# s0phia-/tetris

Hardware: AMD Instinct MI355X
Metric: env-steps/sec (higher is better)
Workload: dtype u32; 1 GPU; 1048576 envs/GPU x 1 GPU, 10x20 board, pieces=default, uniform random valid actions, in-kernel auto-reset, device bag seed 0; envs_per_gpu=1048576, observation_output=True, env_steps_per_launch=1, steps_per_graph_replay=1, streams_per_gpu=1, board=10x20, pieces=default, backend=single, device=cuda

## Files before the change

### tetris_amd/csrc/tetris_core.hpp

```cpp
#pragma once
#include <stdint.h>

#if defined(__HIPCC__)
#include <hip/hip_runtime.h>
#define TET_HD __host__ __device__ __forceinline__
#else
#define TET_HD inline
#endif

#ifndef TET_ABLATE
#define TET_ABLATE 0
#endif
#ifndef TET_BAG_SMALL_PATH
#define TET_BAG_SMALL_PATH 1
#endif
#ifndef TET_RESCUE_SKIP
#define TET_RESCUE_SKIP 1
#endif

#ifndef TET_FENCE_EVERY
#define TET_FENCE_EVERY 2
#endif
#ifndef TET_FENCE_MASK
#define TET_FENCE_MASK 1
#endif
#if defined(__HIP_DEVICE_COMPILE__)
#define TET_SCHED_FENCE() __builtin_amdgcn_sched_barrier(0)
#define TET_PIN(x) asm volatile("" : "+v"(x))
#else
#define TET_SCHED_FENCE() ((void)0)
#define TET_PIN(x) ((void)0)
#endif

#if defined(__HIP_DEVICE_COMPILE__)
#define TET_WAVE_ANY(x) (__ballot((x)) != 0ull)
#else
#define TET_WAVE_ANY(x) (x)
#endif

#if defined(__HIP_DEVICE_COMPILE__)
#define TET_SCRATCH_OR(ptr, v) ((void)__hip_atomic_fetch_or((ptr), (v), __ATOMIC_RELAXED, __HIP_MEMORY_SCOPE_WORKGROUP))
#else
#define TET_SCRATCH_OR(ptr, v) (*(ptr) |= (v))
#endif

#if defined(__HIP_DEVICE_COMPILE__)
#define TET_FMUL(a, b) __fmul_rn((a), (b))
#define TET_FADD(a, b) __fadd_rn((a), (b))
#else
#define TET_FMUL(a, b) ((float)((volatile float)(a) * (b)))
#define TET_FADD(a, b) ((float)((volatile float)(a) + (b)))
#endif

namespace tet {

constexpr int kMaxPieces = 12;
constexpr int kMaxCols = 12;
constexpr int kNumCatalogue = 9;

struct Orient {
  int w, H, b[4], n[4];
  bool exists;
};

TET_HD Orient unpack_orient(uint32_t d) {
  Orient o;
  o.w = d & 7;
  o.H = (d >> 3) & 7;
#pragma unroll
  for (int j = 0; j < 4; ++j) {
    o.b[j] = (d >> (6 + 5 * j)) & 3;
    o.n[j] = (d >> (8 + 5 * j)) & 7;
  }
  o.exists = (d >> 31) != 0;
  return o;
}

#ifndef TET_NO_PACK
#define TET_NO_PACK 0
#endif
TET_HD constexpr bool board_packed(int word_bytes, int num_rows) { return !TET_NO_PACK && num_rows + 4 <= 6 * word_bytes; }
TET_HD constexpr int n_planes(int C, bool packed) { return packed ? (C / 4) * 3 + ((C % 4) * 3 + 3) / 4 : C; }
constexpr int kTileEnvs = 64;
TET_HD constexpr int64_t plane_index(int64_t i, int p, int NP) { return ((i >> 6) * NP + p) * kTileEnvs + (i & 63); }
TET_HD constexpr int64_t board_words(int64_t B, int NP) { return ((B + kTileEnvs - 1) / kTileEnvs) * NP * kTileEnvs; }

template <typename W, int C, bool PACK>
TET_HD void unpack_board(const W (&w)[n_planes(C, PACK)], W (&col)[C]) {
  if (!PACK) {
#pragma unroll
    for (int c = 0; c < C; ++c) col[c] = w[c < n_planes(C, PACK) ? c : 0];
    return;
  }
  constexpr int Wb = 8 * (int)sizeof(W), F = Wb * 3 / 4, P = n_planes(C, PACK);
  const W M = (W)(((W)1 << F) - 1);
#pragma unroll
  for (int g = 0; 4 * g < C; ++g) {
    const int b = 3 * g, c0 = 4 * g;
    const W w0 = w[b], w1 = w[b + 1 < P ? b + 1 : b], w2 = w[b + 2 < P ? b + 2 : b];
    col[c0] = (W)(w0 & M);
    if (c0 + 1 < C) col[c0 + 1] = (W)(((w0 >> F) | (w1 << (Wb - F))) & M);
    if (c0 + 2 < C) col[c0 + 2] = (W)(((w1 >> (2 * F - Wb)) | (w2 << (2 * Wb - 2 * F))) & M);
    if (c0 + 3 < C) col[c0 + 3] = (W)(w2 >> (3 * F - 2 * Wb));
  }
}

template <typename W, int C, bool PACK>
TET_HD void pack_board(const W (&col)[C], W (&w)[n_planes(C, PACK)]) {
  if (!PACK) {
#pragma unroll
    for (int c = 0; c < n_planes(C, PACK); ++c) w[c] = col[c < C ? c : 0];
    return;
  }
  constexpr int Wb = 8 * (int)sizeof(W), F = Wb * 3 / 4, P = n_planes(C, PACK);
#pragma unroll
  for (int g = 0; 4 * g < C; ++g) {
    const int b = 3 * g, c0 = 4 * g;
    const W x0 = col[c0], x1 = c0 + 1 < C ? col[c0 + 1 < C ? c0 + 1 : c0] : (W)0;
    const W x2 = c0 + 2 < C ? col[c0 + 2 < C ? c0 + 2 : c0] : (W)0, x3 = c0 + 3 < C ? col[c0 + 3 < C ? c0 + 3 : c0] : (W)0;
    w[b] = (W)(x0 | (x1 << F));
    if (b + 1 < P) w[b + 1 < P ? b + 1 : b] = (W)((x1 >> (Wb - F)) | (x2 << (2 * F - Wb)));
    if (b + 2 < P) w[b + 2 < P ? b + 2 : b] = (W)((x2 >> (2 * Wb - 2 * F)) | (x3 << (3 * F - 2 * Wb)));
  }
}

template <typename W, int C, bool PACK>
TET_HD void load_board(const W* planes, int64_t , int64_t i, W (&col)[C]) {
  constexpr int NP = n_planes(C, PACK);
  W w[NP];
  const W* rec = planes + plane_index(i, 0, NP);
#pragma unroll
  for (int p = 0; p < NP; ++p) w[p] = rec[p * kTileEnvs];
  unpack_board<W, C, PACK>(w, col);
}
template <typename W, int C, bool PACK>
TET_HD void store_board(W* planes, int64_t , int64_t i, const W (&col)[C]) {
  constexpr int NP = n_planes(C, PACK);
  W w[NP];
  pack_board<W, C, PACK>(col, w);
  W* rec = planes + plane_index(i, 0, NP);
#pragma unroll
  for (int p = 0; p < NP; ++p) rec[p * kTileEnvs] = w[p];
}

template <typename W>
TET_HD W load_column_rt(const W* planes, int64_t , int64_t i, int c, int C, bool packed) {
  const int NP = n_planes(C, packed);
  if (!packed) return planes[plane_index(i, c, NP)];
  constexpr int Wb = 8 * (int)sizeof(W), F = Wb * 3 / 4;
  const W M = (W)(((W)1 << F) - 1);
  const int b = 3 * (c >> 2), k = c & 3;
  const W lo = planes[plane_index(i, b + (k == 0 ? 0 : k - 1), NP)];
  if (k == 0) return (W)(lo & M);
  if (k == 3) return (W)(lo >> (3 * F - 2 * Wb));
  const W hi = planes[plane_index(i, b + k, NP)];
  return k == 1 ? (W)(((lo >> F) | (hi << (Wb - F))) & M) : (W)(((lo >> (2 * F - Wb)) | (hi << (2 * Wb - 2 * F))) & M);
}
template <typename W>
TET_HD void store_columns_rt(W* planes, int64_t , int64_t i, const W* col, int C, bool packed) {
  if (!packed) {
    for (int c = 0; c < C; ++c) planes[plane_index(i, c, C)] = col[c];
    return;
  }
  constexpr int Wb = 8 * (int)sizeof(W), F = Wb * 3 / 4;
  const int P = n_planes(C, true);
  for (int p = 0; p < P; ++p) {
    const int c0 = 4 * (p / 3), q = p % 3;
    const W a = c0 + q < C ? col[c0 + q] : (W)0, b = c0 + q + 1 < C ? col[c0 + q + 1] : (W)0;
    const W v = q == 0 ? (W)(a | (b << F))
                       : (q == 1 ? (W)((a >> (Wb - F)) | (b << (2 * F - Wb))) : (W)((a >> (2 * Wb - 2 * F)) | (b << (3 * F - 2 * Wb))));
    planes[plane_index(i, p, P)] = v;
  }
}

constexpr uint64_t kMaskBits = (1ull << 48) - 1;
constexpr int kFieldStride = 12;
TET_HD constexpr int mask_bit(int k, int c) { return kFieldStride * k + c; }
TET_HD uint64_t meta_pack(uint64_t mask, int piece, uint32_t bag) {
  return (mask & kMaskBits) | ((uint64_t)(piece & 15) << 48) | ((uint64_t)(bag & 0xFFF) << 52);
}
TET_HD uint64_t meta_mask(uint64_t m) { return m & kMaskBits; }
TET_HD int meta_piece(uint64_t m) { return (int)((m >> 48) & 15); }
TET_HD uint32_t meta_bag(uint64_t m) { return (uint32_t)(m >> 52); }

TET_HD int popc(uint32_t x) { return __builtin_popcount(x); }
TET_HD int popc(uint64_t x) { return __builtin_popcountll(x); }
TET_HD int bitlen(uint32_t x) { return 31 - __builtin_clz((x << 1) | 1u); }
TET_HD int bitlen(uint64_t x) { return 63 - __builtin_clzll((x << 1) | 1ull); }
template <typename W>
TET_HD W lowmask(int n) { return (W)(((W)1 << n) - 1); }

TET_HD uint32_t mix32(uint32_t x) {
  x ^= x >> 16;
  x *= 0x7feb352dU;
  x ^= x >> 15;
  x *= 0x846ca68bU;
  x ^= x >> 16;
  return x;
}
TET_HD uint32_t hash_key(uint64_t seed, uint64_t counter) {
  uint32_t k = mix32((uint32_t)seed ^ 0x9E3779B9U);
  k = mix32(k ^ (uint32_t)(seed >> 32));
  k = mix32(k ^ (uint32_t)counter);
  k = mix32(k ^ (uint32_t)(counter >> 32));
  return k;
}
TET_HD uint32_t hash_env(uint32_t key, uint32_t env) {
  uint32_t h = (key ^ env) * 0x9E3779B1U;
  h ^= h >> 16;
  h *= 0x85EBCA6BU;
  h ^= h >> 13;
  return h;
}
TET_HD int scale16(uint32_t r16, int n) { return (int)((r16 * (uint32_t)n) >> 16); }

TET_HD int select_bit32(uint32_t v, int k) {
  int pos = 0;
  int c = popc(v & 0xFFFFu);
  if (k >= c) { k -= c; pos += 16; v >>= 16; }
  c = popc(v & 0xFFu);
  if (k >= c) { k -= c; pos += 8; v >>= 8; }
  c = popc(v & 0xFu);
  if (k >= c) { k -= c; pos += 4; v >>= 4; }
  c = popc(v & 0x3u);
  if (k >= c) { k -= c; pos += 2; v >>= 2; }
  c = (int)(v & 1u);
  if (k >= c) { pos += 1; }
  return pos;
}
TET_HD int bag_draw(uint32_t& bag, int n_pieces, uint32_t r16) {
  if (bag == 0) bag = (1u << n_pieces) - 1u;
  const int k = scale16(r16, popc(bag));
  uint32_t v = bag;
  int pos = 0;
  int c = popc(v & 0xFFu);
  if (k >= c) { pos = 8; v >>= 8; }
  int kk = k >= c ? k - c : k;
  c = popc(v & 0xFu);
  if (kk >= c) { kk -= c; pos += 4; v >>= 4; }
  c = popc(v & 0x3u);
  if (kk >= c) { kk -= c; pos += 2; v >>= 2; }
  c = (int)(v & 1u);
  if (kk >= c) pos += 1;
  bag &= ~(1u << pos);
  return pos;
}

TET_HD int bag_draw_lut(uint32_t& bag, int n_pieces, uint32_t r16, const uint8_t* sel_nib) {
  if (bag == 0) bag = (1u << n_pieces) - 1u;
#if TET_BAG_SMALL_PATH
  if (n_pieces <= 4) {
    const int k4 = scale16(r16, popc(bag));
    const int pos4 = (int)sel_nib[bag * 4u + (uint32_t)k4];
    bag &= ~(1u << pos4);
    return pos4;
  }
#endif
  int k = scale16(r16, popc(bag));
  const int c0 = popc(bag & 0xFu), c1 = c0 + popc(bag & 0xF0u);
  const int grp = (k >= c0) + (k >= c1);
  k -= grp == 0 ? 0 : (grp == 1 ? c0 : c1);
  const uint32_t nib = (bag >> (4 * grp)) & 15u;
  const int pos = 4 * grp + (int)sel_nib[nib * 4u + (uint32_t)k];
  bag &= ~(1u << pos);
  return pos;
}

struct alignas(16) OrientEntry {
  uint32_t sh[4];
  uint32_t rj0[2];
  uint32_t rj1[2];
  uint32_t vert4;
  uint32_t desc;
  uint32_t pad_[2];
};
static_assert(sizeof(OrientEntry) == 48, "table staging and LDS reads assume 48-byte entries");

struct SetTable {
  OrientEntry orient[kMaxPieces][4];
  uint64_t fullmask[kMaxPieces];
};

TET_HD const OrientEntry* piece_entries(const SetTable& tab, int np) {
  uint32_t off = (uint32_t)np * (uint32_t)sizeof(tab.orient[0]);
  TET_PIN(off);
  return reinterpret_cast<const OrientEntry*>(reinterpret_cast<const char*>(&tab.orient[0][0]) + off);
}

template <int CR>
struct LutLayout {
  static constexpr int kHoleEntries = 1 << (CR + 1), kWellsEntries = 1 << CR;
  static constexpr int kHoleA = 0, kHoleU = kHoleEntries, kWellsS = 2 * kHoleEntries;
  static constexpr int kWellsLead = kWellsS + kWellsEntries, kWellsTrail = kWellsLead + kWellsEntries;
  static constexpr int kSelPair = kWellsTrail + kWellsEntries, kSelNib = kSelPair + 256 * 8;
  static constexpr int kBytes = kSelNib + 16 * 4;
};
constexpr int kFeatureLutBytes = LutLayout<12>::kBytes;
constexpr int kFeatureLut10Bytes = LutLayout<10>::kBytes;
struct AfterLut {
  static constexpr int kHoleA = LutLayout<12>::kHoleA, kHoleU = LutLayout<12>::kHoleU;
  static constexpr int kWellsPack = 2 * LutLayout<12>::kHoleEntries;
  static constexpr int kSelPair = kWellsPack + 4 * LutLayout<12>::kWellsEntries, kSelNib = kSelPair + 256 * 8;
  static constexpr int kBytes = kSelNib + 16 * 4;
};
constexpr int kAfterLutBytes = AfterLut::kBytes;

TET_HD uint32_t spread2(uint32_t x) {
  x = (x | (x << 8)) & 0x00FF00FFu;
  x = (x | (x << 4)) & 0x0F0F0F0Fu;
  x = (x | (x << 2)) & 0x33333333u;
  x = (x | (x << 1)) & 0x55555555u;
  return x;
}

template <int C>
TET_HD uint32_t mask_field(uint64_t mask, int k) { return (uint32_t)(mask >> (kFieldStride * k)) & ((1u << C) - 1u); }

template <int C>
TET_HD void slot_of_action_lut(uint64_t mask, int k, const uint8_t* sel_pair, int& kk, int& c) {
  static_assert(C <= 12, "three 4-column groups per 12-bit field");
  constexpr uint32_t kLoopBits = (1u << (2 * kFieldStride)) - 1u;
  const uint32_t w0 = (uint32_t)mask & kLoopBits, w1 = (uint32_t)(mask >> (2 * kFieldStride)) & kLoopBits;
  const int n0 = popc(w0);
  const bool second = k >= n0;
  const uint32_t w = second ? w1 : w0;
  int kr = second ? k - n0 : k;
  constexpr uint32_t kG0 = 0xFu | (0xFu << kFieldStride);
  const int c0 = popc(w & kG0), c1 = c0 + popc(w & (kG0 << 4));
  const int grp = (C > 4 ? (kr >= c0) : 0) + (C > 8 ? (kr >= c1) : 0);
  kr -= grp == 0 ? 0 : (grp == 1 ? c0 : c1);
  const uint32_t t = w >> (4 * grp);
  const uint32_t idx = (t & 15u) | (((t >> kFieldStride) & 15u) << 4);
  const uint32_t r = sel_pair[idx * 8u + (uint32_t)kr];
  c = 4 * grp + (int)(r & 3u);
  kk = (second ? 2 : 0) + (int)(r >> 2);
}
template <int C>
TET_HD void slot_of_action(uint64_t mask, int k, int& kk, int& c) {
  const uint32_t f0 = mask_field<C>(mask, 0), f1 = mask_field<C>(mask, 1);
  const uint32_t f2 = mask_field<C>(mask, 2), f3 = mask_field<C>(mask, 3);
  const int n0 = popc(f0) + popc(f1);
  const bool second = k >= n0;
  const uint32_t z = spread2(second ? f2 : f0) | (spread2(second ? f3 : f1) << 1);
  const int pos = select_bit32(z, second ? k - n0 : k);
  c = pos >> 1;
  kk = (second ? 2 : 0) + (pos & 1);
}
template <int C>
TET_HD int row_of_slot(uint64_t mask, int kk, int c) {
  const int L = kk >> 1;
  const uint32_t fa = mask_field<C>(mask, 2 * L), fb = mask_field<C>(mask, 2 * L + 1);
  const uint32_t below = (1u << c) - 1u;
  int row = popc(fa & below) + popc(fb & below) + ((kk & 1) ? (int)((fa >> c) & 1u) : 0);
  if (L) row += popc(mask_field<C>(mask, 0)) + popc(mask_field<C>(mask, 1));
  return row;
}

template <typename W, int C>
TET_HD void heights_of(const W (&col)[C], int (&h)[C]) {
#pragma unroll
  for (int c = 0; c < C; ++c) h[c] = bitlen(col[c]);
}

template <typename W, int C>
TET_HD int stamp_static(const W (&col)[C], const int (&h)[C], int c, const Orient& o, W (&nb)[C],
                        W (&pbits)[4]) {
  int a = -64;
#pragma unroll
  for (int j = 0; j < 4; ++j)
    if (c + j < C) {
      int v = (j < o.w) ? h[c + j] - o.b[j] : -64;
      a = v > a ? v : a;
    }
  if (a < 0) a = 0;
#pragma unroll
  for (int i = 0; i < C; ++i) nb[i] = col[i];
#pragma unroll
  for (int j = 0; j < 4; ++j) {
    int nj = (j < o.w) ? o.n[j] : 0;
    pbits[j] = (W)(lowmask<W>(nj) << (a + o.b[j]));
    if (c + j < C) nb[c + j] |= pbits[j];
  }
  return a;
}

template <typename W, int C>
TET_HD int clear_lines(W (&col)[C], const W (&pbits)[4], int a, int* eroded_cells) {
  W F = (W)((W)~(W)0 << a);
#pragma unroll
  for (int i = 0; i < C; ++i) F &= col[i];
  int k = popc(F);
  int er = 0;
  if (F != 0) {
#pragma unroll
    for (int j = 0; j < 4; ++j) er += popc((W)(F & pbits[j]));
    while (F != 0) {
      int p = bitlen(F) - 1;
      W low = lowmask<W>(p);
#pragma unroll
      for (int i = 0; i < C; ++i) col[i] = (W)((col[i] & low) | ((col[i] >> (p + 1)) << p));
      F = (W)(F & low);
    }
  }
  *eroded_cells = er;
  return k;
}

template <typename W, int NCH = 0, int CR = 12>
TET_HD void col_own(W x, int hi, int R, const uint8_t* lut, W& ho, int& nh, int& f1, int& f7) {
  ho = (W)(~x & lowmask<W>(hi));
  nh = popc(ho);
  const uint8_t* lut_a = lut + LutLayout<CR>::kHoleA;
  const uint8_t* lut_u = lut + LutLayout<CR>::kHoleU;
  int d7 = 0, u = 0;
  if (!(TET_ABLATE & 16)) {
#pragma unroll
    for (int k = 0; CR * k < (int)(8 * sizeof(W)) - 1; ++k) {
      if (NCH > 0 ? k < NCH : (k < 2 || CR * k < R + 4)) {
        const uint32_t up = (uint32_t)(x >> (CR * k));
        const uint32_t idx = (NCH > 0 && k == NCH - 1) ? up : (up & (uint32_t)(LutLayout<CR>::kHoleEntries - 1));
        const int uk = lut_u[idx];
        u += uk;
        d7 += lut_a[idx];
        const bool more = NCH > 0 ? k + 1 < NCH : (CR * (k + 1) < R + 4);
        if (CR * (k + 1) < (int)(8 * sizeof(W)) && more) d7 += uk * popc((W)(x >> (CR * (k + 1))));
      }
    }
  }
  f1 = 2 * u;
  f7 = d7;
}

template <typename W>
TET_HD int col_rowtrans(W x, W L, int hi, int hL, int nh_left) {
  const int dl = hL - hi;
  return popc((W)((x ^ L) & lowmask<W>(hi))) + (dl > 0 ? dl : 0) - ((hi == 0) ? nh_left : 0);
}

template <typename W, int NCH = 0, int CR = 12>
TET_HD int col_wells(W x, W L, W Rr, int hi, int R, bool left_wall, bool right_wall, const uint8_t* lut) {
  W w = (W)(~x & L & Rr);
  if (left_wall || right_wall) w = (W)(w & lowmask<W>(hi > R ? hi : R));
  const uint8_t* lut_s = lut + LutLayout<CR>::kWellsS;
  const uint8_t* lut_lead = lut + LutLayout<CR>::kWellsLead;
  const uint8_t* lut_trail = lut + LutLayout<CR>::kWellsTrail;
  int total = 0, carry = 0;
#pragma unroll
  for (int k = 0; CR * k < (int)(8 * sizeof(W)) - 1; ++k) {
    if (NCH > 0 ? k < NCH : (k < 2 || CR * k < R + 4)) {
      const uint32_t up = (uint32_t)(w >> (CR * k));
      const uint32_t idx = (NCH > 0 && k == NCH - 1) ? up : (up & (uint32_t)(LutLayout<CR>::kWellsEntries - 1));
      const bool last = NCH > 0 && k == NCH - 1;
      total += lut_s[idx];
      if (k == 0) {
        if (!last) carry = lut_trail[idx];
      } else {
        const int lead = lut_lead[idx];
        total += carry * lead;
        if (!last) {
          const int trail = lut_trail[idx];
          carry = (lead == CR) ? carry + CR : trail;
        }
      }
    }
  }
  return (TET_ABLATE & 32) ? 0 : total;
}

template <typename W, int NCH = 0>
TET_HD int col_wells_packed(W x, W L, W Rr, int hi, int R, bool left_wall, bool right_wall, const uint32_t* pack) {
  constexpr int CR = 12;
  W w = (W)(~x & L & Rr);
  if (left_wall || right_wall) w = (W)(w & lowmask<W>(hi > R ? hi : R));
  uint32_t total = 0, carry = 0;
#pragma unroll
  for (int k = 0; CR * k < (int)(8 * sizeof(W)) - 1; ++k) {
    if (NCH > 0 ? k < NCH : (k < 2 || CR * k < R + 4)) {
      const uint32_t up = (uint32_t)(w >> (CR * k));
      const bool last = NCH > 0 && k == NCH - 1;
      const uint32_t e = pack[last ? up : (up & 4095u)];
      total += e & 0xFFFFu;
      const uint32_t lead = e >> 24, trail = (e >> 16) & 255u;
      if (k == 0) {
        if (!last) carry = trail;
      } else {
        total += carry * lead;
        if (!last) carry = (lead == (uint32_t)CR) ? carry + (uint32_t)CR : trail;
      }
    }
  }
  return (int)total;
}

template <typename W, int C, int NCH = 0, int CR = 12, bool PACKW = false>
TET_HD void board_features(const W (&col)[C], const int (&h)[C], int R, const uint8_t* hole_lut,
                           int& rows_with_holes, int& col_trans, int& holes, int& wells, int& row_trans,
                           int& hole_depth) {
  const W wall = lowmask<W>(R + 4);
  W hole_rows = 0;
  int f1 = C;
  int f2 = 0, f4 = 0, f7 = 0;
  int f5 = R - popc(col[C - 1]);
  int nh_left = 0;
#pragma unroll
  for (int i = 0; i < C; ++i) {
    const W L = (i == 0) ? wall : col[i - 1];
    const W Rr = (i == C - 1) ? wall : col[i + 1];
    const int hL = (i == 0) ? R : h[i - 1];
    W ho;
    int nh, d1, d7;
    col_own<W, NCH, CR>(col[i], h[i], R, hole_lut, ho, nh, d1, d7);
    f1 += d1;
    f2 += nh;
    f7 += d7;
    hole_rows |= ho;
    f5 += col_rowtrans<W>(col[i], L, h[i], hL, nh_left);
    nh_left = nh;
    if (PACKW)
      f4 += col_wells_packed<W, NCH>(col[i], L, Rr, h[i], R, i == 0, i == C - 1,
                                     reinterpret_cast<const uint32_t*>(hole_lut + AfterLut::kWellsPack));
    else
      f4 += col_wells<W, NCH, CR>(col[i], L, Rr, h[i], R, i == 0, i == C - 1, hole_lut);
    if (TET_FENCE_EVERY > 0 && i % TET_FENCE_EVERY == TET_FENCE_EVERY - 1 && i + 1 < C) {
      TET_PIN(f1);
      TET_PIN(f2);
      TET_PIN(f4);
      TET_PIN(f5);
      TET_PIN(f7);
      TET_SCHED_FENCE();
    }
  }
  rows_with_holes = popc(hole_rows);
  col_trans = f1;
  holes = f2;
  wells = f4;
  row_trans = f5;
  hole_depth = f7;
}

template <typename W, int C, int NCH = 0, int CR = 12, bool PACKW = false>
TET_HD void bcts_features(const W (&col)[C], const int (&h)[C], int R, const uint8_t* hole_lut, int anchor_row,
                          int H, int eroded_cells, int n_cleared, float (&f)[8]) {
  int f0, f1, f2, f4, f5, f7;
  board_features<W, C, NCH, CR, PACKW>(col, h, R, hole_lut, f0, f1, f2, f4, f5, f7);
  f[0] = (float)f0;
  f[1] = (float)f1;
  f[2] = (float)f2;
  f[3] = (float)anchor_row + 0.5f * (float)(H - 1) + 1.0f;
  f[4] = (float)f4;
  f[5] = (float)f5;
  f[6] = (float)(eroded_cells * n_cleared);
  f[7] = (float)f7;
}

TET_HD constexpr int level_stride(int C) { return C <= 10 ? 10 : 12; }
template <int C> struct MissBits { typedef uint32_t type; };
template <> struct MissBits<11> { typedef uint64_t type; };
template <> struct MissBits<12> { typedef uint64_t type; };
TET_HD int ctz_any(uint32_t x) { return __builtin_ctz(x); }
TET_HD int ctz_any(uint64_t x) { return __builtin_ctzll(x); }

template <typename W, int C>
TET_HD uint64_t valid_mask(const W (&col)[C], const int (&h)[C], const OrientEntry* tab, uint64_t fullmask, int R) {
  static_assert(C <= 12, "four 12-bit level fields + one empty field fill the 64-bit level word; 12-bit mask fields");
  constexpr int LS = level_stride(C);
  typedef typename MissBits<C>::type FT;
  uint32_t P[3] = {0u, 0u, 0u};
#pragma unroll
  for (int c = 0; c < C; ++c) P[c >> 2] |= (uint32_t)h[c] << (8 * (c & 3));
  uint32_t lv[4];
#pragma unroll
  for (int l = 1; l <= 4; ++l) {
    const uint32_t K = (uint32_t)(127 - (R - l)) * 0x01010101u;
    uint32_t g = 0;
#pragma unroll
    for (int q = 0; q < (C + 3) / 4; ++q)
      g |= ((((P[q] + K) & 0x80808080u) * 0x00204081u) >> 28) << (4 * q);
    lv[l - 1] = g;
  }
  const uint64_t Z = ((uint64_t)lv[0] << LS) | ((uint64_t)lv[1] << (2 * LS)) | ((uint64_t)lv[2] << (3 * LS)) |
                     ((uint64_t)lv[3] << (4 * LS));
  const bool rescue = !TET_RESCUE_SKIP || TET_WAVE_ANY(popc(lv[2]) >= C - 4);
  uint32_t X[3] = {0u, 0u, 0u}, Y[3] = {0u, 0u, 0u};
  uint32_t rv1 = 0, rv2 = 0;
  if (rescue) {
    FT Fall = 0;
#pragma unroll
    for (int c = 0; c < C; ++c) Fall |= (FT)((uint32_t)(col[c] >> (R - 3)) & 7u) << (3 * c);
    const FT Mall = (FT)~Fall;
    constexpr FT kEveryThird = (FT)0x9249249249249249ull & (FT)(((FT)1 << (3 * C)) - 1);
    constexpr FT kTop = (FT)1 << (8 * sizeof(FT) - 1);
#pragma unroll
    for (int t = 0; t < 3; ++t) {
      const FT m = (FT)(Mall >> t) & kEveryThird;
      const int lo = (ctz_any((FT)(m | kTop)) * 11) >> 5;
      const int hi = ((bitlen((FT)(m | 1)) - 1) * 11) >> 5;
      X[t] = ~0u << hi;
      Y[t] = m ? (2u << lo) - 1u : 0u;
    }
    const uint32_t s0 = X[0] & Y[0], s1 = X[1] & Y[1], s2 = X[2] & Y[2];
    rv1 = s0 | s1 | s2;
    rv2 = s1 & s2;
  }
  const uint32_t cm = (1u << C) - 1u;
  uint64_t mask = 0;
#pragma unroll
  for (int k = 0; k < 4; ++k) {
    const OrientEntry& e = tab[k];
    uint32_t r = 0;
#pragma unroll
    for (int j = 0; j < 4; ++j) r |= (uint32_t)(Z >> e.sh[j]);
    const uint32_t i1 = r >> LS, i2 = r;
    uint32_t v = ~i1;
    if (rescue) {
      uint32_t r1 = ((X[1] >> e.rj1[0]) & (Y[1] >> e.rj0[0])) | ((X[2] >> e.rj1[1]) & (Y[2] >> e.rj0[1]));
      r1 = (rv1 & e.vert4) | (r1 & ~e.vert4);
      const uint32_t r2 = rv2 & e.vert4;
      v |= ~(i2 & ~r2) & r1;
    }
    mask |= (uint64_t)(v & cm) << (kFieldStride * k);
  }
  return mask & fullmask;
}

template <typename W, int C>
TET_HD int stamp_dynamic(W (&col)[C], const int (&h)[C], int c, uint32_t d, W (&pbits)[4]) {
  static_assert(C <= 12, "heights are packed into three 32-bit words");
  uint32_t P[4] = {0u, 0u, 0u, 0u};
#pragma unroll
  for (int i = 0; i < C; ++i) P[i >> 2] |= (uint32_t)h[i] << (8 * (i & 3));
  const int kq = c >> 2;
  const uint32_t plo = kq == 0 ? P[0] : (kq == 1 ? P[1] : P[2]);
  const uint32_t phi = kq == 0 ? P[1] : (kq == 1 ? P[2] : P[3]);
  const uint32_t win = (uint32_t)((((uint64_t)phi << 32) | plo) >> (8 * (c & 3)));
  const int w = d & 7;
  int a = 0;
#pragma unroll
  for (int j = 0; j < 4; ++j) {
    const int bj = (d >> (6 + 5 * j)) & 3;
    const int v = (int)((win >> (8 * j)) & 255u) - bj;
    a = (j < w && v > a) ? v : a;
  }
#pragma unroll
  for (int j = 0; j < 4; ++j) {
    const int bj = (d >> (6 + 5 * j)) & 3;
    const int nj = (j < w) ? (int)((d >> (8 + 5 * j)) & 7) : 0;
    pbits[j] = (W)(lowmask<W>(nj) << (a + bj));
  }
#pragma unroll
  for (int i = 0; i < C; ++i) {
    W add = 0;
#pragma unroll
    for (int j = 0; j < 4; ++j)
      if (i - j >= 0) add |= (W)(pbits[j] & (W)(0 - (W)(c == i - j)));
    col[i] |= add;
  }
  return a;
}

template <typename W, int C>
TET_HD int stamp_scratch(W (&col)[C], W* scratch, int sstride, int c, uint32_t d, W (&pbits)[4]) {
#pragma unroll
  for (int i = 0; i < C; ++i) scratch[i * sstride] = col[i];
  const int w = d & 7;
  int a = 0;
  int idx[4];
#pragma unroll
  for (int j = 0; j < 4; ++j) {
    idx[j] = (c + j < C ? c + j : C - 1) * sstride;
    const int bj = (d >> (6 + 5 * j)) & 3;
    const int v = bitlen(scratch[idx[j]]) - bj;
    a = (j < w && v > a) ? v : a;
  }
#pragma unroll
  for (int j = 0; j < 4; ++j) {
    const int bj = (d >> (6 + 5 * j)) & 3;
    const int nj = (int)((d >> (8 + 5 * j)) & 7);
    pbits[j] = (W)(lowmask<W>(nj) << (a + bj));
    TET_SCRATCH_OR(&scratch[idx[j]], pbits[j]);
  }
#pragma unroll
  for (int i = 0; i < C; ++i) col[i] = scratch[i * sstride];
  return a;
}

template <typename W, int C, int NCH, typename Emit>
TET_HD void afterstates_env(const W (&col)[C], uint64_t meta, const SetTable& tab, const uint8_t* lut, int R,
                            Emit&& emit) {
  const uint32_t* pack = reinterpret_cast<const uint32_t*>(lut + AfterLut::kWellsPack);
  int h[C];
  heights_of<W, C>(col, h);
  const W wall = lowmask<W>(R + 4);
  const int piece = meta_piece(meta);
  const uint64_t full = tab.fullmask[piece];
  W HO[C];
  uint32_t D[C];
  int sF1 = C;
  int sHoles = 0, sF7 = 0, sWells = 0;
  int sRT = R - popc(col[C - 1]);
  {
    int nh_left = 0;
#pragma unroll
    for (int i = 0; i < C; ++i) {
      const W L = (i == 0) ? wall : col[i - 1];
      const W Rr = (i == C - 1) ? wall : col[i + 1];
      const int hL = (i == 0) ? R : h[i - 1];
      int nh, e1, e7;
      col_own<W, NCH, 12>(col[i], h[i], R, lut, HO[i], nh, e1, e7);
      const int e5 = col_rowtrans<W>(col[i], L, h[i], hL, nh_left);
      const int e4 = col_wells_packed<W, NCH>(col[i], L, Rr, h[i], R, i == 0, i == C - 1, pack);
      nh_left = nh;
      D[i] = (uint32_t)(e1 >> 1) | ((uint32_t)nh << 5) | ((uint32_t)e5 << 11) | ((uint32_t)e4 << 18);
      sF1 += e1;
      sHoles += nh;
      sF7 += e7;
      sRT += e5;
      sWells += e4;
    }
  }
  uint64_t slow = 0;
  const uint64_t valid = meta_mask(meta) & full;
  int row_all = 0, row_valid = 0;
#pragma unroll 1
  for (int L = 0; L < 2; ++L) {
    const uint32_t d0 = tab.orient[piece][2 * L].desc, d1 = tab.orient[piece][2 * L + 1].desc;
    if (!TET_WAVE_ANY((d0 | d1) >> 31)) continue;
    const int wu0_ = 1 + (TET_WAVE_ANY((d0 & 7u) > 1) ? 1 : 0) + (TET_WAVE_ANY((d0 & 7u) > 2) ? 1 : 0) +
                    (TET_WAVE_ANY((d0 & 7u) > 3) ? 1 : 0);
    const int wu1_ = 1 + (TET_WAVE_ANY((d1 & 7u) > 1) ? 1 : 0) + (TET_WAVE_ANY((d1 & 7u) > 2) ? 1 : 0) +
                    (TET_WAVE_ANY((d1 & 7u) > 3) ? 1 : 0);
    const int wu0 = (TET_ABLATE & 1024) ? 4 : wu0_, wu1 = (TET_ABLATE & 1024) ? 4 : wu1_;
    const uint32_t fe0 = mask_field<C>(full, 2 * L), fe1 = mask_field<C>(full, 2 * L + 1);
    const uint32_t fv0 = mask_field<C>(valid, 2 * L), fv1 = mask_field<C>(valid, 2 * L + 1);
    uint32_t sl0 = 0, sl1 = 0;
#pragma unroll
    for (int c = 0; c < C; ++c) {
      W a_ex = (W)~(W)0, o_ex = 0;
#pragma unroll
      for (int i = 0; i < C; ++i)
        if (i < c || i > c + 3) {
          a_ex &= col[i];
          o_ex |= HO[i];
        }

#pragma unroll
      for (int oi = 0; oi < 2; ++oi) {
        const int k = 2 * L + oi;
        const uint32_t dsc = oi ? d1 : d0;
        const int wu = oi ? wu1 : wu0;
        const int wd = (int)(dsc & 7u), H = (int)((dsc >> 3) & 7u);
        const bool ex = ((oi ? fe1 : fe0) >> c) & 1u;
        if (!(TET_ABLATE & 512) && !TET_WAVE_ANY(ex)) continue;
        const bool is_valid = ((oi ? fv1 : fv0) >> c) & 1u;
        const int my_row_all = row_all, my_row_valid = row_valid;
        row_all += ex ? 1 : 0;
        row_valid += is_valid ? 1 : 0;
        int a = 0;
#pragma unroll
        for (int j = 0; j < 4; ++j)
          if (c + j < C) {
            const int v = h[c + j] - (int)((dsc >> (6 + 5 * j)) & 3u);
            a = (j < wd && v > a) ? v : a;
          }
        W XN[6];
        int HN[6], NHN[5];
        {
          const int cm1 = c >= 1 ? c - 1 : 0, c4 = c + 4 < C ? c + 4 : C - 1;
          XN[0] = (c >= 1) ? col[cm1] : wall;
          HN[0] = (c >= 1) ? h[cm1] : R;
          NHN[0] = (c >= 1) ? (int)((D[cm1] >> 5) & 63u) : 0;
          XN[5] = (c + 4 < C) ? col[c4] : wall;
          HN[5] = (c + 4 < C) ? h[c4] : R;
        }
        W hrows = o_ex, F = a_ex;
        int dholes = 0, dtops = 0, df7 = 0, dlast = 0;
#pragma unroll
        for (int j = 0; j < 4; ++j) {
          constexpr int kz = 0;
          const int i = c + j < C ? c + j : kz;
          if (c + j < C) {
            const int bj = (int)((dsc >> (6 + 5 * j)) & 3u), nj = (int)((dsc >> (8 + 5 * j)) & 7u);
            const int bot = (j < wd) ? a + bj : h[i];
            const int g = bot - h[i];
            XN[j + 1] = (W)(col[i] | (W)(lowmask<W>(nj) << bot));
            HN[j + 1] = bot + nj;
            hrows |= (W)(HO[i] | (W)(lowmask<W>(g) << h[i]));
            const int top = g > 0 ? 1 : 0;
            dholes += g;
            dtops += top;
            df7 += ((int)(D[i] & 31u) + top) * nj;
            NHN[j + 1] = (int)((D[i] >> 5) & 63u) + g;
            if (c + j == C - 1) dlast = nj;
          } else {
            XN[j + 1] = wall;
            HN[j + 1] = R;
            NHN[j + 1] = 0;
          }
          F &= XN[j + 1];
        }
        F &= (W)((W)~(W)0 << a);
        const bool fast = ex && F == 0;
        if (ex && F != 0) (oi ? sl1 : sl0) |= 1u << c;
        if (!(TET_ABLATE & 512) && !TET_WAVE_ANY(fast)) continue;
        int drt = 0;
#pragma unroll
        for (int q = 1; q <= 5; ++q)
          if (c + q - 1 < C && q <= wu + 1) {
            constexpr int kz = 0;
            const int i = c + q - 1 < C ? c + q - 1 : kz;
            drt += col_rowtrans<W>(XN[q], XN[q - 1], HN[q], HN[q - 1], NHN[q - 1]) - (int)((D[i] >> 11) & 127u);
          }
        int dwells = 0;
#pragma unroll
        for (int q = 0; q <= 5; ++q)
          if (c + q - 1 >= 0 && c + q - 1 < C && q <= wu + 1) {
            constexpr int kz = 0;
            const int i = (c + q - 1 >= 0 && c + q - 1 < C) ? c + q - 1 : kz;
            const int il = (i - 1 >= 0) ? i - 1 : kz, ir = (i + 1 < C) ? i + 1 : C - 1;
            const W Lq = (q >= 1) ? XN[q - 1] : ((i >= 1) ? col[il] : wall);
            const W Rq = (q <= 4) ? XN[q + 1] : ((i + 1 < C) ? col[ir] : wall);
            dwells += col_wells_packed<W, NCH>(XN[q], Lq, Rq, HN[q], R, i == 0, i == C - 1, pack) - (int)(D[i] >> 18);
          }
        float f[8];
        f[0] = (float)popc(hrows);
        f[1] = (float)(sF1 + 2 * dtops);
        f[2] = (float)(sHoles + dholes);
        f[3] = (float)a + 0.5f * (float)(H - 1) + 1.0f;
        f[4] = (float)(sWells + dwells);
        f[5] = (float)(sRT + drt - dlast);
        f[6] = 0.0f;
        f[7] = (float)(sF7 + df7);
        emit(fast, k, c, f, my_row_all, my_row_valid, is_valid);
        TET_SCHED_FENCE();
      }
    }
    slow |= ((uint64_t)sl0 << mask_bit(2 * L, 0)) | ((uint64_t)sl1 << mask_bit(2 * L + 1, 0));
  }
  while (TET_WAVE_ANY(slow != 0) && !(TET_ABLATE & 256)) {
    const bool has = slow != 0;
    const int sb = has ? bitlen(slow) - 1 : 0;
    slow &= ~(1ull << sb);
    W fb[C];
#pragma unroll
    for (int i = 0; i < C; ++i) fb[i] = col[i];
    W pbits[4];
    int fh[C];
    const int sk = sb / kFieldStride, sc = sb - sk * kFieldStride;
    const uint32_t od = tab.orient[piece][sk].desc;
    const int aa = stamp_dynamic<W, C>(fb, h, sc, od, pbits);
    int eroded = 0;
    const int kk = clear_lines<W, C>(fb, pbits, aa, &eroded);
    heights_of<W, C>(fb, fh);
    float f[8];
    bcts_features<W, C, NCH, 12, true>(fb, fh, R, lut, aa, (int)((od >> 3) & 7u), eroded, kk, f);
    emit(has, sk, sc, f, row_of_slot<C>(full, sk, sc), row_of_slot<C>(valid, sk, sc), ((valid >> sb) & 1) != 0);
  }
}

TET_HD float fitness_of(const float (&f)[8], const float (&w)[8]) {
#if defined(__clang__)
#pragma clang fp contract(off)
#endif
  float acc = TET_FMUL(f[0], w[0]);
#pragma unroll
  for (int q = 1; q < 8; ++q) acc = TET_FADD(acc, TET_FMUL(f[q], w[q]));
  return acc;
}

struct StepOut {
  float obs[8];
  int action;
  int reward;
  int done;
  int lines;
  int n_valid;
  int piece;
  int invalid;
};

struct StepCfg {
  int R;
  int n_pieces;
  int auto_reset;
  uint32_t key_step;
  uint32_t key_policy;
  int compute_obs;
  float direct_by[8];
  int has_direct_by;
};

TET_HD int policy_random(uint32_t key_policy, uint32_t env, int n_valid) {
  return scale16(hash_env(key_policy, env) >> 16, n_valid);
}

template <typename W, int C, int NCH = 0, int CR = 12, bool PACKW = false>
TET_HD void env_step(W (&col)[C], uint64_t& meta, int action, bool use_policy, const SetTable& tab,
                     const uint8_t* hole_lut, W* scratch, int sstride, const StepCfg& cfg, uint32_t env, int draw,
                     int draw_reset, StepOut& out) {
  const int R = cfg.R;
  const uint64_t mask = meta_mask(meta);
  int piece = meta_piece(meta);
  uint32_t bag = meta_bag(meta);
  const int nv = popc(mask);
  if (use_policy) action = policy_random(cfg.key_policy, env, nv);
  out.action = action;
  out.invalid = (action < 0 || action >= nv) ? 1 : 0;
  if (out.invalid) {
#pragma unroll
    for (int k = 0; k < 8; ++k) out.obs[k] = 0.0f;
    out.reward = 0;
    out.done = (nv == 0) ? 1 : 0;
    out.lines = 0;
    out.n_valid = nv;
    out.piece = piece;
    return;
  }
  int sk, c;
  slot_of_action_lut<C>(mask, action, hole_lut + (PACKW ? AfterLut::kSelPair : LutLayout<CR>::kSelPair), sk, c);
  const uint32_t od = tab.orient[piece][sk].desc;
  const int oH = (od >> 3) & 7;

  int h[C];
  W pbits[4];
  const int a = stamp_scratch<W, C>(col, scratch, sstride, c, od, pbits);
  int eroded = 0;
  const int k = (TET_ABLATE & 8) ? 0 : clear_lines<W, C>(col, pbits, a, &eroded);
  heights_of<W, C>(col, h);
  if ((TET_ABLATE & 1) || !cfg.compute_obs) {
#pragma unroll
    for (int i = 0; i < 8; ++i) out.obs[i] = (float)h[i < C ? i : C - 1];
  } else
  bcts_features<W, C, NCH, CR, PACKW>(col, h, R, hole_lut, a, oH, eroded, k, out.obs);
  if (cfg.has_direct_by) {
#pragma unroll
    for (int i = 0; i < 8; ++i) out.obs[i] *= cfg.direct_by[i];
  }
  const uint32_t rnd = hash_env(cfg.key_step, env);
  const uint8_t* sel_nib = hole_lut + (PACKW ? AfterLut::kSelNib : LutLayout<CR>::kSelNib);
  int np = draw >= 0 ? draw : bag_draw_lut(bag, cfg.n_pieces, rnd >> 16, sel_nib);
  uint64_t nmask = (TET_ABLATE & 2) ? (tab.fullmask[np] ^ (uint64_t)h[0])
                                    : valid_mask<W, C>(col, h, piece_entries(tab, np), tab.fullmask[np], R);
  int nnv = popc(nmask);
  int done = nnv == 0;
  out.reward = k - 1 + (done ? -100 : 0);
  out.done = done;
  out.lines = k;
  if (done && cfg.auto_reset) {
#pragma unroll
    for (int i = 0; i < C; ++i) col[i] = 0;
    np = draw_reset >= 0 ? draw_reset : bag_draw_lut(bag, cfg.n_pieces, rnd & 0xFFFFu, sel_nib);
    nmask = tab.fullmask[np];
    nnv = popc(nmask);
  }
  out.n_valid = nnv;
  out.piece = np;
  meta = meta_pack(nmask, np, bag);
}

template <typename W, int C, int NCH = 0>
TET_HD int rollout_env(const W (&col0)[C], uint64_t meta0, int a0, int length, int policy, const float (&w)[8],
                       const SetTable& tab, const uint8_t* hole_lut, W* scratch, int sstride, int R, int n_pieces,
                       uint32_t key0, uint32_t uid, const uint8_t* fed = nullptr) {
  W col[C];
#pragma unroll
  for (int i = 0; i < C; ++i) col[i] = col0[i];
  uint64_t meta = meta0;
  if (popc(meta_mask(meta)) == 0) return -1;
  StepCfg cfg;
  cfg.R = R;
  cfg.n_pieces = n_pieces;
  cfg.auto_reset = 0;
  cfg.has_direct_by = 0;
  cfg.compute_obs = 0;
#pragma unroll
  for (int i = 0; i < 8; ++i) cfg.direct_by[i] = 1.0f;
  int ret = 0;
#pragma unroll 1
  for (int t = 0; t < length; ++t) {
    cfg.key_step = mix32(key0 + 2u * (uint32_t)t);
    cfg.key_policy = mix32(key0 + 2u * (uint32_t)t + 1u);
    int action = a0;
    bool use_policy = false;
    if (t > 0) {
      if (policy == 0) {
        use_policy = true;
        action = -1;
      } else {
        float best = 0.f;
        int best_row = -1;
        afterstates_env<W, C, NCH>(col, meta, tab, hole_lut, R, [&](bool has, int, int, float (&f)[8], int, int row, bool is_valid) {
          if (!has) return;
          if (is_valid) {
            const float v = fitness_of(f, w);
            if (best_row < 0 || v > best || (v == best && row < best_row)) {
              best = v;
              best_row = row;
            }
          }
        });
        action = best_row;
      }
    }
    StepOut out;
    env_step<W, C, NCH, 12, true>(col, meta, action, use_policy, tab, hole_lut, scratch, sstride, cfg, uid,
                                  fed ? (int)fed[t] : -1, -1, out);
    if (out.done || out.invalid) return -1;
    if (t > 0) ret += out.reward;
  }
  return ret;
}

}
```

### tetris_amd/csrc/tetris_table.hpp

```cpp
#pragma once
#include <string.h>

#include "../../include/tetris_hip.h"
#include "tetris_core.hpp"

namespace tet {

struct CatOrient { int w; int b[4]; int n[4]; };
struct CatPiece { int n_orient[2]; CatOrient o[2][2]; };

static const CatPiece kCatalogue[TETRIS_N_CATALOGUE] = {
    {{1, 1}, {{{1, {0}, {4}}}, {{4, {0, 0, 0, 0}, {1, 1, 1, 1}}}}},
    {{1, 0}, {{{2, {0, 0}, {2, 2}}}}},
    {{1, 1}, {{{3, {0, 0, 1}, {1, 2, 1}}}, {{2, {1, 0}, {2, 2}}}}},
    {{1, 1}, {{{1, {0}, {3}}}, {{3, {0, 0, 0}, {1, 1, 1}}}}},
    {{2, 2}, {{{2, {0, 0}, {1, 2}}, {2, {0, 1}, {2, 1}}}, {{2, {1, 0}, {1, 2}}, {2, {0, 0}, {2, 1}}}}},
    {{1, 1}, {{{3, {1, 0, 0}, {1, 2, 1}}}, {{2, {0, 1}, {2, 2}}}}},
    {{2, 2}, {{{3, {0, 0, 0}, {1, 2, 1}}, {3, {1, 0, 1}, {1, 2, 1}}}, {{2, {1, 0}, {1, 3}}, {2, {0, 1}, {3, 1}}}}},
    {{2, 2}, {{{3, {0, 0, 0}, {1, 1, 2}}, {3, {0, 1, 1}, {2, 1, 1}}}, {{2, {2, 0}, {1, 3}}, {2, {0, 0}, {3, 1}}}}},
    {{2, 2}, {{{3, {0, 0, 0}, {2, 1, 1}}, {3, {1, 1, 0}, {1, 1, 2}}}, {{2, {0, 2}, {3, 1}}, {2, {0, 0}, {1, 3}}}}},
};

inline uint32_t pack_orient(const CatOrient& o) {
  int H = 0;
  uint32_t d = (uint32_t)o.w;
  for (int j = 0; j < o.w; ++j) {
    if (o.b[j] + o.n[j] > H) H = o.b[j] + o.n[j];
    d |= (uint32_t)o.b[j] << (6 + 5 * j);
    d |= (uint32_t)o.n[j] << (8 + 5 * j);
  }
  d |= (uint32_t)H << 3;
  d |= 1u << 31;
  return d;
}

inline int n_placements(int pid, int C) {
  const CatPiece& p = kCatalogue[pid];
  int total = 0;
  for (int l = 0; l < 2; ++l)
    if (p.n_orient[l] > 0 && C - p.o[l][0].w + 1 > 0) total += (C - p.o[l][0].w + 1) * p.n_orient[l];
  return total;
}

inline void pack_mask_fields(const CatOrient& o, OrientEntry* e, int C) {
  const int LS = level_stride(C);
  int H = 0;
  for (int j = 0; j < o.w; ++j)
    if (o.b[j] + o.n[j] > H) H = o.b[j] + o.n[j];
  for (int j = 0; j < o.w; ++j) e->sh[j] = (uint32_t)(LS * (H - o.b[j] - 1) + j);
  for (int j = o.w; j < 4; ++j) e->sh[j] = e->sh[0];
  e->vert4 = (o.w == 1 && H == 4) ? ~0u : 0u;
  for (int t = 1; t < 3; ++t) {
    const int rho = t - 4 + H;
    e->rj0[t - 1] = 31;
    e->rj1[t - 1] = 0;
    if (rho < 0 || rho > H - 2) continue;
    int j0 = -1, j1 = -1;
    for (int j = 0; j < o.w; ++j)
      if (o.b[j] <= rho && rho < o.b[j] + o.n[j]) {
        if (j0 < 0) j0 = j;
        j1 = j;
      }
    e->rj0[t - 1] = (uint32_t)j0;
    e->rj1[t - 1] = (uint32_t)j1;
  }
}

inline void build_table(const TetrisDesc* d, SetTable* t) {
  memset(t, 0, sizeof(*t));
  const int C = d->num_columns;
  for (int i = 0; i < d->n_pieces; ++i) {
    const CatPiece& p = kCatalogue[d->piece_ids[i]];
    uint64_t full = 0;
    for (int l = 0; l < 2; ++l)
      for (int oi = 0; oi < p.n_orient[l]; ++oi) {
        OrientEntry* e = &t->orient[i][l * 2 + oi];
        e->desc = pack_orient(p.o[l][oi]);
        pack_mask_fields(p.o[l][oi], e, C);
        for (int c = 0; c + p.o[l][oi].w <= C; ++c) full |= 1ull << mask_bit(2 * l + oi, c);
      }
    t->fullmask[i] = full;
  }
}

#ifndef TET_COLUMNS
#define TET_COLUMNS(X) X(5) X(6) X(7) X(8) X(9) X(10) X(11) X(12)
#endif

inline bool columns_supported(int C) {
  switch (C) {
#define TET_X(CC) case CC:
    TET_COLUMNS(TET_X)
#undef TET_X
    return true;
    default:
      return false;
  }
}

inline const char* error_text(int code) {
  switch (code) {
    case TETRIS_OK: return "ok";
    case TETRIS_E_NULL: return "required pointer is NULL";
    case TETRIS_E_DESC: return "descriptor not initialised by tetris_hip_desc_init or inconsistent";
    case TETRIS_E_COLUMNS: return "num_columns not compiled into libtetris_hip";
    case TETRIS_E_ROWS: return "num_rows outside [4, 59]";
    case TETRIS_E_PIECES: return "bad piece list";
    case TETRIS_E_BATCH: return "batch size must be positive";
    case TETRIS_E_STREAM: return "replay stream needs cursor and stream_len > 0";
    case TETRIS_E_STRIDE: return "afterstate strides must be multiples of 4 floats and >= 8";
    default: return nullptr;
  }
}

inline int check_desc(const TetrisDesc* d) {
  if (!d) return TETRIS_E_NULL;
  if (d->abi_version != TETRIS_HIP_ABI_VERSION) return TETRIS_E_DESC;
  if (d->num_rows < 4 || d->num_rows > 59) return TETRIS_E_ROWS;
  if (d->word_bytes != ((d->num_rows + 4 <= 31) ? 4 : 8)) return TETRIS_E_DESC;
  if (d->n_pieces < 1 || d->n_pieces > TETRIS_MAX_PIECES) return TETRIS_E_PIECES;
  for (int i = 0; i < d->n_pieces; ++i)
    if (d->piece_ids[i] < 0 || d->piece_ids[i] >= TETRIS_N_CATALOGUE) return TETRIS_E_PIECES;
  return TETRIS_OK;
}


inline int desc_init(TetrisDesc* desc, int32_t num_columns, int32_t num_rows, const int32_t* piece_ids,
                     int32_t n_pieces, const float* direct_by) {
  if (!desc || !piece_ids) return TETRIS_E_NULL;
  memset(desc, 0, sizeof(*desc));
  if (!columns_supported(num_columns)) return TETRIS_E_COLUMNS;
  if (num_rows < 4 || num_rows > 59) return TETRIS_E_ROWS;
  if (n_pieces < 1 || n_pieces > TETRIS_MAX_PIECES) return TETRIS_E_PIECES;
  desc->abi_version = TETRIS_HIP_ABI_VERSION;
  desc->num_columns = num_columns;
  desc->num_rows = num_rows;
  desc->word_bytes = (num_rows + 4 <= 31) ? 4 : 8;
  desc->n_pieces = n_pieces;
  int amax = 0;
  for (int i = 0; i < n_pieces; ++i) {
    if (piece_ids[i] < 0 || piece_ids[i] >= TETRIS_N_CATALOGUE) return TETRIS_E_PIECES;
    desc->piece_ids[i] = piece_ids[i];
    int n = n_placements(piece_ids[i], num_columns);
    if (n > amax) amax = n;
  }
  desc->a_max = amax;
  if (direct_by) {
    desc->has_direct_by = 1;
    for (int i = 0; i < 8; ++i) desc->direct_by[i] = direct_by[i];
  }
  return TETRIS_OK;
}

}
```

Measured before the change: 35.64 billion env-steps/s.

## Build valid-mask level words directly from top board rows for narrow 32-bit boards

For 32-bit boards of up to ten columns, valid_mask now builds its per-level occupancy words by gathering the top four rows of each column with multiply-based bit interleaving, instead of comparing packed column heights against each level. The level stride becomes a fixed 16 bits with a reversed level order, and the shift table built on the host is updated to match. The rescue path reads row masks directly instead of the 3-bit-per-column ctz/bitlen scaling. This is meant to cut ALU work in the per-step mask computation, at the risk of subtle bit-layout correctness errors.

After: 37.32 billion env-steps/s, median of 6. 4.7% higher.

```diff
diff --git a/tetris_amd/csrc/tetris_core.hpp b/tetris_amd/csrc/tetris_core.hpp
--- a/tetris_amd/csrc/tetris_core.hpp
+++ b/tetris_amd/csrc/tetris_core.hpp
@@ -553,56 +553,94 @@
   f[7] = (float)f7;
 }
 
-TET_HD constexpr int level_stride(int C) { return C <= 10 ? 10 : 12; }
+constexpr int kLevelStride = 16;
 template <int C> struct MissBits { typedef uint32_t type; };
 template <> struct MissBits<11> { typedef uint64_t type; };
 template <> struct MissBits<12> { typedef uint64_t type; };
 TET_HD int ctz_any(uint32_t x) { return __builtin_ctz(x); }
 TET_HD int ctz_any(uint64_t x) { return __builtin_ctzll(x); }
 
-template <typename W, int C>
+template <typename W, int C, bool TOP = false>
 TET_HD uint64_t valid_mask(const W (&col)[C], const int (&h)[C], const OrientEntry* tab, uint64_t fullmask, int R) {
-  static_assert(C <= 12, "four 12-bit level fields + one empty field fill the 64-bit level word; 12-bit mask fields");
-  constexpr int LS = level_stride(C);
+  static_assert(C <= 12, "16-bit level fields; 12-bit mask fields");
+  static_assert(!TOP || (sizeof(W) == 4 && C <= 10), "the top-rows form is written for 32-bit boards of up to ten columns");
+  constexpr int LS = kLevelStride;
   typedef typename MissBits<C>::type FT;
-  uint32_t P[3] = {0u, 0u, 0u};
-#pragma unroll
-  for (int c = 0; c < C; ++c) P[c >> 2] |= (uint32_t)h[c] << (8 * (c & 3));
-  uint32_t lv[4];
-#pragma unroll
-  for (int l = 1; l <= 4; ++l) {
-    const uint32_t K = (uint32_t)(127 - (R - l)) * 0x01010101u;
-    uint32_t g = 0;
-#pragma unroll
-    for (int q = 0; q < (C + 3) / 4; ++q)
-      g |= ((((P[q] + K) & 0x80808080u) * 0x00204081u) >> 28) << (4 * q);
-    lv[l - 1] = g;
-  }
-  const uint64_t Z = ((uint64_t)lv[0] << LS) | ((uint64_t)lv[1] << (2 * LS)) | ((uint64_t)lv[2] << (3 * LS)) |
-                     ((uint64_t)lv[3] << (4 * LS));
-  const bool rescue = !TET_RESCUE_SKIP || TET_WAVE_ANY(popc(lv[2]) >= C - 4);
+  const uint32_t cm = (1u << C) - 1u;
+  uint32_t zlo, zhi;
+  uint32_t b3;
+  uint32_t mrow[3] = {0u, 0u, 0u};
+  if constexpr (TOP) {
+    uint32_t lo = 0, hi = 0;
+#pragma unroll
+    for (int g = 0; g < 4 && g < C; ++g) {
+      uint32_t pk = (uint32_t)(col[g] >> (R - 4));
+      uint32_t sel = 1u;
+      if (g + 4 < C) { pk |= (uint32_t)(col[g + 4] >> (R - 4)) << 4; sel |= 1u << 4; }
+      if (g + 8 < C) { pk |= (uint32_t)(col[g + 8] >> (R - 4)) << 8; sel |= 1u << 8; }
+      const uint32_t u = pk * (0x8001u << g);
+      const uint32_t mk = (sel * 0x10001u) << g;
+      lo |= u & mk;
+      hi |= (u >> 2) & mk;
+    }
+    zhi = hi | (hi >> 16);
+    zlo = lo | (lo >> 16) | ((zhi & 0xFFFFu) * 0x10001u);
+    b3 = zlo >> 16;
+    mrow[0] = ~(lo >> 16) & cm;
+    mrow[1] = ~hi & cm;
+    mrow[2] = ~(hi >> 16) & cm;
+  } else {
+    uint32_t P[3] = {0u, 0u, 0u};
+#pragma unroll
+    for (int c = 0; c < C; ++c) P[c >> 2] |= (uint32_t)h[c] << (8 * (c & 3));
+    uint32_t lv[4];
+#pragma unroll
+    for (int l = 1; l <= 4; ++l) {
+      const uint32_t K = (uint32_t)(127 - (R - l)) * 0x01010101u;
+      uint32_t g = 0;
+#pragma unroll
+      for (int q = 0; q < (C + 3) / 4; ++q)
+        g |= ((((P[q] + K) & 0x80808080u) * 0x00204081u) >> 28) << (4 * q);
+      lv[l - 1] = g;
+    }
+    zlo = lv[3] | (lv[2] << LS);
+    zhi = lv[1] | (lv[0] << LS);
+    b3 = lv[2];
+  }
+  const uint64_t Z = ((uint64_t)zhi << 32) | zlo;
+  const bool rescue = !TET_RESCUE_SKIP || TET_WAVE_ANY(popc(b3) >= C - 4);
   uint32_t X[3] = {0u, 0u, 0u}, Y[3] = {0u, 0u, 0u};
   uint32_t rv1 = 0, rv2 = 0;
   if (rescue) {
-    FT Fall = 0;
-#pragma unroll
-    for (int c = 0; c < C; ++c) Fall |= (FT)((uint32_t)(col[c] >> (R - 3)) & 7u) << (3 * c);
-    const FT Mall = (FT)~Fall;
-    constexpr FT kEveryThird = (FT)0x9249249249249249ull & (FT)(((FT)1 << (3 * C)) - 1);
-    constexpr FT kTop = (FT)1 << (8 * sizeof(FT) - 1);
-#pragma unroll
-    for (int t = 0; t < 3; ++t) {
-      const FT m = (FT)(Mall >> t) & kEveryThird;
-      const int lo = (ctz_any((FT)(m | kTop)) * 11) >> 5;
-      const int hi = ((bitlen((FT)(m | 1)) - 1) * 11) >> 5;
-      X[t] = ~0u << hi;
-      Y[t] = m ? (2u << lo) - 1u : 0u;
+    if constexpr (TOP) {
+#pragma unroll
+      for (int t = 0; t < 3; ++t) {
+        const uint32_t m = mrow[t];
+        const int lo = __builtin_ctz(m | 0x80000000u);
+        const int hi = bitlen((uint32_t)(m | 1u)) - 1;
+        X[t] = ~0u << hi;
+        Y[t] = m ? (2u << lo) - 1u : 0u;
+      }
+    } else {
+      FT Fall = 0;
+#pragma unroll
+      for (int c = 0; c < C; ++c) Fall |= (FT)((uint32_t)(col[c] >> (R - 3)) & 7u) << (3 * c);
+      const FT Mall = (FT)~Fall;
+      constexpr FT kEveryThird = (FT)0x9249249249249249ull & (FT)(((FT)1 << (3 * C)) - 1);
+      constexpr FT kTop = (FT)1 << (8 * sizeof(FT) - 1);
+#pragma unroll
+      for (int t = 0; t < 3; ++t) {
+        const FT m = (FT)(Mall >> t) & kEveryThird;
+        const int lo = (ctz_any((FT)(m | kTop)) * 11) >> 5;
+        const int hi = ((bitlen((FT)(m | 1)) - 1) * 11) >> 5;
+        X[t] = ~0u << hi;
+        Y[t] = m ? (2u << lo) - 1u : 0u;
+      }
     }
     const uint32_t s0 = X[0] & Y[0], s1 = X[1] & Y[1], s2 = X[2] & Y[2];
     rv1 = s0 | s1 | s2;
     rv2 = s1 & s2;
   }
-  const uint32_t cm = (1u << C) - 1u;
   uint64_t mask = 0;
 #pragma unroll
   for (int k = 0; k < 4; ++k) {
@@ -610,7 +648,7 @@
     uint32_t r = 0;
 #pragma unroll
     for (int j = 0; j < 4; ++j) r |= (uint32_t)(Z >> e.sh[j]);
-    const uint32_t i1 = r >> LS, i2 = r;
+    const uint32_t i1 = r, i2 = r >> LS;
     uint32_t v = ~i1;
     if (rescue) {
       uint32_t r1 = ((X[1] >> e.rj1[0]) & (Y[1] >> e.rj0[0])) | ((X[2] >> e.rj1[1]) & (Y[2] >> e.rj0[1]));
@@ -939,7 +977,7 @@
   const uint8_t* sel_nib = hole_lut + (PACKW ? AfterLut::kSelNib : LutLayout<CR>::kSelNib);
   int np = draw >= 0 ? draw : bag_draw_lut(bag, cfg.n_pieces, rnd >> 16, sel_nib);
   uint64_t nmask = (TET_ABLATE & 2) ? (tab.fullmask[np] ^ (uint64_t)h[0])
-                                    : valid_mask<W, C>(col, h, piece_entries(tab, np), tab.fullmask[np], R);
+                                    : valid_mask<W, C, (sizeof(W) == 4 && C <= 10)>(col, h, piece_entries(tab, np), tab.fullmask[np], R);
   int nnv = popc(nmask);
   int done = nnv == 0;
   out.reward = k - 1 + (done ? -100 : 0);
diff --git a/tetris_amd/csrc/tetris_table.hpp b/tetris_amd/csrc/tetris_table.hpp
--- a/tetris_amd/csrc/tetris_table.hpp
+++ b/tetris_amd/csrc/tetris_table.hpp
@@ -42,12 +42,12 @@
   return total;
 }
 
-inline void pack_mask_fields(const CatOrient& o, OrientEntry* e, int C) {
-  const int LS = level_stride(C);
+inline void pack_mask_fields(const CatOrient& o, OrientEntry* e) {
+  const int LS = kLevelStride;
   int H = 0;
   for (int j = 0; j < o.w; ++j)
     if (o.b[j] + o.n[j] > H) H = o.b[j] + o.n[j];
-  for (int j = 0; j < o.w; ++j) e->sh[j] = (uint32_t)(LS * (H - o.b[j] - 1) + j);
+  for (int j = 0; j < o.w; ++j) e->sh[j] = (uint32_t)(LS * (4 - (H - o.b[j])) + j);
   for (int j = o.w; j < 4; ++j) e->sh[j] = e->sh[0];
   e->vert4 = (o.w == 1 && H == 4) ? ~0u : 0u;
   for (int t = 1; t < 3; ++t) {
@@ -76,7 +76,7 @@
       for (int oi = 0; oi < p.n_orient[l]; ++oi) {
         OrientEntry* e = &t->orient[i][l * 2 + oi];
         e->desc = pack_orient(p.o[l][oi]);
-        pack_mask_fields(p.o[l][oi], e, C);
+        pack_mask_fields(p.o[l][oi], e);
         for (int c = 0; c + p.o[l][oi].w <= C; ++c) full |= 1ull << mask_bit(2 * l + oi, c);
       }
     t->fullmask[i] = full;
```
